# egorchistov/color-transfer

Measured on AMD Instinct MI355X. Metric: stereopairs/s at 1920×1080 (linear + dcmcs3di fwd), 1/2/4/8 GPU, higher is better.
Workload: dtype f32 (float32 I/O; float32 difference forms in both sweeps, float64 only in the per-frame statistics records); 1 GPU; configs[1]: methods.linear.color_transfer_between_images (Reinhard) on 1920x1080 synthetic float32 RGB pairs, HBM-resident; float32 arithmetic in both sweeps (difference forms, Lab within 5e-5 of the float64 reference; gate 1e-4); + per-frame psnr against resident ground truth; io_dtype=float32, height=1080, width=1920, lab_arithmetic=table

## Files before the change

color-transfer_amd/csrc/attention16.hip:

```cpp
#include <hip/hip_runtime.h>
#include <cstdint>
#include <cmath>
#include "ct_attention16.h"
#include "ct_env.h"
#include "ct_split16.h"

namespace ct {

static constexpr float kLog2eH = 1.4426950408889634f, kLn2H = 0.6931471805599453f;

constexpr int kSsRowH(int C) { return 2 * C + 16; }

__device__ __forceinline__ void xcd_order(int &bx, int &by) {
    bx = blockIdx.x; by = blockIdx.y;
    if (gridDim.z != 1) return;
    const unsigned int gx = gridDim.x, total = gx * gridDim.y, lin = by * gx + bx, full = total & ~7u;
    if (lin >= full) return;
    const unsigned int vid = (lin & 7u) * (full >> 3) + (lin >> 3);
    bx = (int)(vid % gx); by = (int)(vid / gx);
}

template <int C, int CV, bool MAP, bool IDX = false>
__global__ __launch_bounds__(256, 2) void attention16_tokens_kernel(const float *__restrict__ q, const float *__restrict__ k,
                                                                    const float *__restrict__ v, const int *__restrict__ region,
                                                                    const int *__restrict__ rowmap, float *__restrict__ out,
                                                                    float *__restrict__ stats, int L, float scale,
                                                                    float *__restrict__ part, long long kv_shift, long long kv_total,
                                                                    float *__restrict__ disp) {
    static_assert(!IDX || !MAP, "the expected index is built for the unmapped rows");
    constexpr bool PVS = CV >= 32;
    constexpr int NVT = PVS ? CV / 32 : 1;
    constexpr int KV4 = (32 * C / 4) / 256;
    constexpr int VV4 = PVS ? (32 * CV / 4) / 256 : 1;
    constexpr int SROW = kSsRowH(C);
    constexpr int VROWB = (CV * 2) % 256 == 0 ? CV * 2 + 64 : CV * 2;
// ... 158 lines not shown
    fetch_rows(jb);
    fetch(jb);
    fetch_rows(jb + 32);
    note_max();
    __syncthreads();
    stage();
    e_cur = e_stage;
    __syncthreads();
    for (int j0 = jb; j0 < je; j0 += 32) {
        const bool more = j0 + 32 < je;
        if (more) {
            fetch(j0 + 32);
            fetch_rows(j0 + 64);
        }
        f32x16 s;
#pragma unroll
        for (int r = 0; r < 16; ++r) s[r] = 0.f;
        {
            const unsigned char *kp = Ks + nl * SROW + 16 * hl;
            uint4 ac[2], an[2];
#pragma unroll
            for (int p = 0; p < 2; ++p) ac[p] = *reinterpret_cast<const uint4 *>(kp + p * 32 * SROW);
#pragma unroll
            for (int st = 0; st < C / 16; ++st) {
                if (st + 1 < C / 16) {
#pragma unroll
                    for (int p = 0; p < 2; ++p) an[p] = *reinterpret_cast<const uint4 *>(kp + p * 32 * SROW + 32 * (st + 1));
                }
                sp16_mfma3(s, ac, qf[st]);
#pragma unroll
                for (int p = 0; p < 2; ++p) ac[p] = an[p];
            }
        }
        const float f = Gs[0] * gq;
        if (region) {
            const float maskv = fmaxf((-100.0f * kLog2eH) * (Gs[1] * sq), -3.0e38f);
            int rk[16];
#pragma unroll
            for (int r = 0; r < 16; ++r) rk[r] = Rs[(r & 3) + 8 * (r >> 2) + 4 * hl];
#pragma unroll
            for (int r = 0; r < 16; ++r) s[r] += (rk[r] != qreg) ? maskv : 0.0f;
        }
        if (j0 + 32 > L) {
#pragma unroll
            for (int r = 0; r < 16; ++r) s[r] = (j0 + (r & 3) + 8 * (r >> 2) + 4 * hl < L) ? s[r] : -INFINITY;
        }
        float mx = s[0];
#pragma unroll
        for (int r = 1; r < 16; ++r) mx = fmaxf(mx, s[r]);
        mx = fmaxf(mx, __shfl_xor(mx, 32, 64));
        const float m_new = fmaxf(m_run, mx * f);
        const float corr = __builtin_amdgcn_exp2f(m_run - m_new);
        const float off = POFF - m_new;
        float psum = 0.f;
#pragma unroll
        for (int r = 0; r < 16; ++r) {
            const float p = __builtin_amdgcn_exp2f(fmaf(s[r], f, off));
            s[r] = p;
            psum += p;
        }
        psum += __shfl_xor(psum, 32, 64);
        l_run = l_run * corr + psum;
        m_run = m_new;
        if constexpr (IDX) {
            const float d0 = (float)(j0 + 4 * hl - qi);
            float asum = 0.f;
#pragma unroll
            for (int r = 0; r < 16; ++r) asum = fmaf(s[r], d0 + (float)((r & 3) + 8 * (r >> 2)), asum);
            asum += __shfl_xor(asum, 32, 64);
            a_run = a_run * corr + asum;
        }
        if constexpr (PVS) {
            const float ce = __builtin_amdgcn_ldexpf(corr, e_stage - e_cur);
            e_cur = e_stage;
#pragma unroll
            for (int j = 0; j < NVT; ++j)
#pragma unroll
                for (int r = 0; r < 16; ++r) o[j][r] *= ce;
            typedef short s16x4h __attribute__((ext_vector_type(4)));
            typedef __attribute__((address_space(3))) s16x4h *lds_s16x4;
            const unsigned char *vb = Vs + (4 * hl + ((lane & 15) >> 2)) * VROWB + (16 * ((lane >> 4) & 1) + 4 * (lane & 3)) * 2;
#pragma unroll
            for (int t = 0; t < 2; ++t) {
                const float x[8] = {s[8 * t], s[8 * t + 1], s[8 * t + 2], s[8 * t + 3], s[8 * t + 4], s[8 * t + 5], s[8 * t + 6], s[8 * t + 7]};
                uint4 pf[2];
                sp16_split2x8(x, pf[0], pf[1]);
#pragma unroll
                for (int j = 0; j < NVT; ++j) {
                    uint4 vf[2];
#pragma unroll
                    for (int p = 0; p < 2; ++p) {
                        const unsigned char *a = vb + (p * 32 + 16 * t) * VROWB + 64 * j;
                        const s16x4h lo = __builtin_amdgcn_ds_read_tr16_b64_v4i16((lds_s16x4)(a));
                        const s16x4h hi = __builtin_amdgcn_ds_read_tr16_b64_v4i16((lds_s16x4)(a + 8 * VROWB));
                        const uint2 l2 = __builtin_bit_cast(uint2, lo), h2 = __builtin_bit_cast(uint2, hi);
                        vf[p] = make_uint4(l2.x, l2.y, h2.x, h2.y);
                    }
                    sp16_mfma3(o[j], vf, pf);
                }
            }
        } else if constexpr (CV == 2) {
            const float *vs2 = reinterpret_cast<const float *>(Vs);
            float ax = 0.f, ay = 0.f;
#pragma unroll
            for (int r = 0; r < 16; ++r) {
                const float2 vv = *reinterpret_cast<const float2 *>(vs2 + ((r & 3) + 8 * (r >> 2) + 4 * hl) * 2);
                ax += s[r] * vv.x;
                ay += s[r] * vv.y;
            }
            ax += __shfl_xor(ax, 32, 64);
            ay += __shfl_xor(ay, 32, 64);
            o2x = o2x * corr + ax;
            o2y = o2y * corr + ay;
        }
        if (more) note_max();
        __syncthreads();
        if (more) {
            stage();
            __syncthreads();
        }
    }
    if (nsplit > 1) {
        float *pp = part + (((size_t)split * gridDim.y + b) * L + qclamp) * (CV + 2);
        if (qlive) {
            if constexpr (PVS) {
#pragma unroll
                for (int j = 0; j < NVT; ++j)
#pragma unroll
                    for (int r = 0; r < 16; ++r) pp[j * 32 + (r & 3) + 8 * (r >> 2) + 4 * hl] = __builtin_amdgcn_ldexpf(o[j][r], -e_cur - (int)POFF);
// ... 14 lines not shown
    }
    if constexpr (PVS) {
        if (qlive) {
            const float ie = __builtin_amdgcn_ldexpf(inv, -e_cur);
            float *op = out + row(qi) * CV;
#pragma unroll
            for (int j = 0; j < NVT; ++j)
#pragma unroll
                for (int r = 0; r < 16; r += 4)
                    *reinterpret_cast<float4 *>(op + j * 32 + 8 * (r >> 2) + 4 * hl) =
                        make_float4(o[j][r] * ie, o[j][r + 1] * ie, o[j][r + 2] * ie, o[j][r + 3] * ie);
        }
    } else if constexpr (CV == 2) {
        if (qlive && hl == 0) *reinterpret_cast<float2 *>(out + row(qi) * 2) = make_float2(o2x * inv, o2y * inv);
    }
}

template <int C>
__global__ __launch_bounds__(256, 2) void attention16_colsum_kernel(const float *__restrict__ q, const float *__restrict__ k,
                                                                    const float *__restrict__ stats, float *__restrict__ colsum, int L,
                                                                    float scale) {
    constexpr int QV4 = (32 * C / 4) / 256;
    constexpr int SROW = kSsRowH(C);
    __shared__ __attribute__((aligned(16))) unsigned char Qs[2 * 32 * SROW];
    __shared__ float2 Ms[32];
    __shared__ __attribute__((aligned(16))) float Mx[4];
    __shared__ float Gs[1];
    const int tid = threadIdx.x, lane = tid & 63, wave = tid >> 6, nl = lane & 31, hl = lane >> 5;
    int bxo, b;
    xcd_order(bxo, b);
// ... 60 lines not shown
            unsigned char *qd = Qs + qq * SROW + 8 * c4;
            *reinterpret_cast<uint2 *>(qd) = make_uint2(h0, h1);
            *reinterpret_cast<uint2 *>(qd + 32 * SROW) = make_uint2(l0, l1);
        }
        if (tid < 32) Ms[tid] = make_float2(mpre.x * kLog2eH, 1.0f / mpre.y);
    };
    float acc = 0.f;
    fetch(0);
    note_max();
    __syncthreads();
    stage();
    __syncthreads();
    for (int i0 = 0; i0 < L; i0 += 32) {
        const bool more = i0 + 32 < L;
        if (more) fetch(i0 + 32);
        f32x16 s;
#pragma unroll
        for (int r = 0; r < 16; ++r) s[r] = 0.f;
        const unsigned char *qp = Qs + nl * SROW + 16 * hl;
        uint4 ac[2], an[2];
#pragma unroll
        for (int p = 0; p < 2; ++p) ac[p] = *reinterpret_cast<const uint4 *>(qp + p * 32 * SROW);
#pragma unroll
        for (int st = 0; st < C / 16; ++st) {
            if (st + 1 < C / 16) {
#pragma unroll
                for (int p = 0; p < 2; ++p) an[p] = *reinterpret_cast<const uint4 *>(qp + p * 32 * SROW + 32 * (st + 1));
            }
            sp16_mfma3(s, ac, kf[st]);
#pragma unroll
            for (int p = 0; p < 2; ++p) ac[p] = an[p];
        }
        const float f = Gs[0] * gk;
        float2 ml[16];
#pragma unroll
        for (int r = 0; r < 16; ++r) ml[r] = Ms[(r & 3) + 8 * (r >> 2) + 4 * hl];
#pragma unroll
        for (int r = 0; r < 16; ++r) acc = fmaf(__builtin_amdgcn_exp2f(fmaf(s[r], f, -ml[r].x)), ml[r].y, acc);
        if (more) note_max();
        __syncthreads();
        if (more) {
            stage();
            __syncthreads();
        }
    }
    acc += __shfl_xor(acc, 32, 64);
    if (hl == 0 && kj < L) colsum[tb + kj] = acc;
}

bool attention16_enabled() {
    static const int on = env_int("CT_HIP_ATT16", 1);
    return on != 0;
}

void attention16_tokens128(const float *q, const float *k, const float *v, const int *region, const int *rowmap, float *out, int batch,
                           int len, int cv, float scale, int nsplit, float *ws, long long kv_shift, long long kv_total, hipStream_t s) {
    dim3 grid((len + 127) / 128, batch, nsplit);
    float *nostats = nullptr;
#define CT_ATT16(CVV, MAPPED) hipLaunchKernelGGL((attention16_tokens_kernel<128, CVV, MAPPED>), grid, dim3(256), 0, s, q, k, v, region, rowmap, out, nostats, len, scale, ws, kv_shift, kv_total, (float *)nullptr)
    if (cv == 128) { if (rowmap) CT_ATT16(128, true); else CT_ATT16(128, false); }
    else { if (rowmap) CT_ATT16(2, true); else CT_ATT16(2, false); }
#undef CT_ATT16
}

void attention16_rows64(const float *q, const float *k, const float *v, float *out, float *stats, int batch, int len, float scale,
                        hipStream_t s) {
    dim3 grid((len + 127) / 128, batch);
    const int *noreg = nullptr;
    if (v) hipLaunchKernelGGL((attention16_tokens_kernel<64, 96, false>), grid, dim3(256), 0, s, q, k, v, noreg, noreg, out, stats, len, scale, (float *)nullptr, 0LL, 0LL, (float *)nullptr);
    else hipLaunchKernelGGL((attention16_tokens_kernel<64, 0, false>), grid, dim3(256), 0, s, q, k, v, noreg, noreg, out, stats, len, scale, (float *)nullptr, 0LL, 0LL, (float *)nullptr);
}

void attention16_rows64_disp(const float *q, const float *k, const float *v, float *out, float *disp, int batch, int len, float scale,
                             hipStream_t s) {
    dim3 grid((len + 127) / 128, batch);
    const int *noreg = nullptr;
    float *nostats = nullptr;
    if (v) hipLaunchKernelGGL((attention16_tokens_kernel<64, 96, false, true>), grid, dim3(256), 0, s, q, k, v, noreg, noreg, out, nostats, len, scale, (float *)nullptr, 0LL, 0LL, disp);
    else hipLaunchKernelGGL((attention16_tokens_kernel<64, 0, false, true>), grid, dim3(256), 0, s, q, k, v, noreg, noreg, out, nostats, len, scale, (float *)nullptr, 0LL, 0LL, disp);
}

void attention16_colsum64(const float *q, const float *k, const float *stats, float *colsum, int batch, int len, float scale, hipStream_t s) {
    dim3 grid((len + 127) / 128, batch);
    hipLaunchKernelGGL((attention16_colsum_kernel<64>), grid, dim3(256), 0, s, q, k, stats, colsum, len, scale);
}

}
```

color-transfer_amd/csrc/attention_tokens.hip:

```cpp
#include "ct_common.h"
#include "ct_split.h"
#include "ct_attention16.h"

namespace ct {

template <bool TO_ROWS>
__global__ __launch_bounds__(256) void rows_transpose_kernel(const float *__restrict__ src, float *__restrict__ dst, int C, int H,
                                                             int W, long long nchw_bstride, int row_channels, int c0) {
    __shared__ float t[32][65];
    const int tid = threadIdx.x;
    const int x0 = blockIdx.x * 64;
    const int by = blockIdx.y, b = by / H, y = by - b * H;
    const size_t plane = (size_t)H * W;
    const float *nsrc = src;
    float *ndst = dst;
    const bool vec = (x0 + 64 <= W) && ((W & 3) == 0) && ((row_channels & 3) == 0) && ((c0 & 3) == 0) && ((nchw_bstride & 3) == 0) &&
                     (((reinterpret_cast<uintptr_t>(src) | reinterpret_cast<uintptr_t>(dst)) & 15) == 0);
    for (int cb = 0; cb < C; cb += 32) {
        const bool full = vec && (cb + 32 <= C);
        if (TO_ROWS) {
            const int c = tid >> 3, xs = (tid & 7) * 8;
            const float *p = nsrc + (size_t)b * nchw_bstride + (size_t)(cb + c) * plane + (size_t)y * W + x0 + xs;
            if (full) {
                const float4 a = reinterpret_cast<const float4 *>(p)[0], bb = reinterpret_cast<const float4 *>(p)[1];
// ... 561 lines not shown
    return CT_OK;
}

int ct_attention_colsum64_f32(const float *q, const float *k, const float *stats, float *colsum, int batch, int len, float scale,
                              void *stream) {
    if (!q || !k || !stats || !colsum || batch < 0 || len < 1) return CT_E_BADARG;
    if ((reinterpret_cast<uintptr_t>(q) | reinterpret_cast<uintptr_t>(k)) & 15) return CT_E_ALIGN;
    if (batch == 0) return CT_OK;
    dim3 grid((len + 127) / 128, batch);
    if (ct::attention16_enabled()) ct::attention16_colsum64(q, k, stats, colsum, batch, len, scale, (hipStream_t)stream);
    else hipLaunchKernelGGL((ct::attention_colsum_kernel<64>), grid, dim3(256), 0, (hipStream_t)stream, q, k, stats, colsum, len, scale);
    CT_CHECK_LAUNCH();
    return CT_OK;
}

}
```

color-transfer_amd/csrc/ct_attention16.h:

```cpp
#pragma once
#include <hip/hip_runtime.h>

namespace ct {

bool attention16_enabled();
void attention16_tokens128(const float *q, const float *k, const float *v, const int *region, const int *rowmap, float *out, int batch,
                           int len, int cv, float scale, int nsplit, float *ws, long long kv_shift, long long kv_total, hipStream_t s);
void attention16_rows64(const float *q, const float *k, const float *v, float *out, float *stats, int batch, int len, float scale,
                        hipStream_t s);
void attention16_rows64_disp(const float *q, const float *k, const float *v, float *out, float *disp, int batch, int len, float scale,
                             hipStream_t s);
void attention16_colsum64(const float *q, const float *k, const float *stats, float *colsum, int batch, int len, float scale, hipStream_t s);

}
```

color-transfer_amd/ct_hip/__init__.py:

```python
from ._core import (ACT_GELU, ACT_LEAKY, ACT_NONE, ACT_RELU, ACT_SIGMOID, ACT_SWISH, ACT_TANH, CT_ABI_VERSION,
                    CT_LAB_STATS_STRIDE, CT_RGB_STATS_STRIDE, CT_WS_IDT, CT_WS_LAB_STATS, CT_WS_REINHARD, CT_WS_REINHARD_PERSIST,
                    CT_WS_REINHARD_PSNR, CT_WS_RGB_MEANCOV, CtHipError, LIB_PATH, SIGNATURES, check, device_status, lib,
                    workspace, _stream)
from .linear import (CT_LAB_EXACT, CT_LAB_TABLE, affine3x3, lab_mode, lab_stats, mk, mk_coef, profile_events, reinhard,
                     reinhard_apply, reinhard_persist, reinhard_persist_supported, reinhard_psnr, reinhard_takes_persist,
                     rgb_meancov, set_lab_mode)
from .metrics import (CT_WS_FSIM, DISTORTIONS, distort_u8, fft2d_, frame_fsim, frame_icid, frame_psnr, frame_ssim, regrain,
                      _fsim_tables)
from .idt import IdtDebug, idt
from .resize_pack import CT_PACK_CHW, CT_PACK_HWC, PACK_LAYOUTS, bicubic_resize, bilinear_resize, pack_u8, resize_geometry
from .packing import (ConvSource, SplitOperands, pack_conv_weight, pack_conv_weight_split, pack_conv_weight_split16,
                      pack_conv_weight_wino16, pack_gconv_weight, pack_linear_weight_split, pack_linear_weight_ws16)
from .gmflow import (convex_upsample, eltwise, fb_check, flow_warp, instance_norm, local_attn_prop, local_corr_flow,
                     local_corr_softmax)
from .conv import (conv2d, conv2d_rows, conv_mode, conv_scratch_prepare, conv_stream_k_state, conv_wino, conv_ws16, gconv2d,
                   s2d_ok, set_conv_mode, set_conv_stream_k, set_conv_wino, set_conv_wino_form, set_conv_ws16, space_to_depth2,
                   _conv_scratch, _conv_split, _sk_cache)
from .linears import layernorm128, linear_layernorm128, linear_tokens, linear_tokens_multi, set_linear_ws16
from .attention import (attention_tokens, nchw_to_rows, nchw_to_tokens, pam_attend, pam_streaming, pam_streaming_rows, pam_valid,
                        pam_valid_rows, tokens_to_nchw)
from .unet import dwconv, gconv2d_pad, scale_planes_, se_gate, upsample2_concat
from .disparity import attention_rows64_index, pam_disp_fill, regress_disp
from .views import (CT_VIEW_ABMSE, CT_VIEW_GRAY, CT_VIEW_LABMSE, CT_VIEW_RGBMSE, abmse_view, chess_mix, flow_to_image, gray_view, labmse_view,
                    rgbmse_view, rgbssim_view)
from .png import INFLATE_STATUS, PNG_MAX_WIDTH, PNG_ROWS_PER_CHUNK, inflate, png_decode, png_deflate, png_geometry
from .augment import AUGMENT_KINDS, AUGMENT_MAX_OPS, AUGMENT_SAMPLE, augment_table, augment_u8, frame_losses
from .pam_losses import PAM_SWEEP_MAX_W, masked_l1_sums, pam_cycle_l1, pam_map_sweep
from . import _core


def __getattr__(name):
    if name == "_lib":
        return _core._lib
    raise AttributeError("module %r has no attribute %r" % (__name__, name))
```

color-transfer_amd/ct_hip/_core.py:

```python
import ctypes
import os
import threading
from typing import NamedTuple

import numpy as np
import torch

_HERE = os.path.dirname(os.path.abspath(__file__))
LIB_PATH = os.environ.get("CT_HIP_LIB") or os.path.join(_HERE, "libct_hip.so")

CT_ABI_VERSION = 9
CT_LAB_STATS_STRIDE = 8
CT_RGB_STATS_STRIDE = 16
CT_WS_LAB_STATS, CT_WS_RGB_MEANCOV, CT_WS_REINHARD, CT_WS_IDT, CT_WS_REINHARD_PSNR, CT_WS_REINHARD_PERSIST = 0, 1, 2, 3, 4, 5

_c_i64 = ctypes.c_int64
_c_int = ctypes.c_int
_c_p = ctypes.c_void_p
_c_sz = ctypes.c_size_t
_c_ll = ctypes.c_longlong
_c_f = ctypes.c_float

ACT_NONE, ACT_LEAKY, ACT_RELU, ACT_SIGMOID, ACT_TANH, ACT_SWISH, ACT_GELU = 0, 1, 2, 3, 4, 5, 6

# ... 18 lines not shown
        with _lock:
            if _lib is None:
                if not os.path.exists(LIB_PATH):
                    raise CtHipError(
                        "HIP library %s not found: build it with `python -c 'import __graft_entry__ as g; g.build()'` "
                        "or `make -C color-transfer_amd/csrc`; this package has no CPU fallback" % LIB_PATH)
                handle = ctypes.CDLL(LIB_PATH)
                for name, (res, args) in SIGNATURES.items():
                    fn = getattr(handle, name)
                    fn.restype = res
                    fn.argtypes = args
                got = handle.ct_abi_version()
                if got != CT_ABI_VERSION:
                    raise CtHipError("%s reports ABI version %d, this binding needs %d: rebuild with `make -C color-transfer_amd/csrc`"
                                     % (LIB_PATH, got, CT_ABI_VERSION))
                _lib = handle
    return _lib


def check(rc):
    if rc != 0:
        raise CtHipError("libct_hip: %s (code %d)" % (lib().ct_error_string(rc).decode(), rc))


def _stream():
    return ctypes.c_void_p(torch.cuda.current_stream().cuda_stream)


def _check_device(t):
    if t.device.index is not None and t.device.index != torch.cuda.current_device():
# ... 117 lines not shown
```

color-transfer_amd/ct_hip/attention.py:

```python
import ctypes

import torch

from ._core import (CtHipError, SIGNATURES, _c_f, _c_int, _c_ll, _c_p, _c_sz, _check_device, _f32c, _nchw_bstride, _opt, _ptr, _stream,
                    check, lib, workspace)

SIGNATURES.update({
    "ct_pam_workspace_bytes": (_c_sz, [_c_int, _c_int, _c_int]),
    "ct_pam_attend_f32": (_c_int, [_c_p, _c_p, _c_p, _c_p, _c_p, _c_p, _c_p, _c_int, _c_int, _c_int, _c_int, _c_int, _c_p]),
    "ct_pam_valid_f32": (_c_int, [_c_p, _c_p, _c_p, _c_p, _c_p, _c_int, _c_int, _c_int, _c_int, _c_p, _c_sz, _c_p]),
    "ct_attention_workspace_bytes": (ctypes.c_size_t, [_c_int, _c_int, _c_int, _c_int]),
    "ct_attention_tokens_f32": (_c_int, [_c_p, _c_p, _c_p, _c_p, _c_p, _c_p, _c_int, _c_int, _c_int, _c_f, _c_int, _c_p,
                                         ctypes.c_size_t, ctypes.c_longlong, _c_p]),
    "ct_nchw_to_rows_f32": (_c_int, [_c_p, _c_p, _c_int, _c_int, _c_int, _c_int, _c_ll, _c_int, _c_int, _c_p]),
    "ct_rows_to_nchw_f32": (_c_int, [_c_p, _c_p, _c_int, _c_int, _c_int, _c_int, _c_ll, _c_int, _c_int, _c_p]),
    "ct_attention_rows64_f32": (_c_int, [_c_p, _c_p, _c_p, _c_p, _c_p, _c_int, _c_int, _c_f, _c_p]),
    "ct_attention_colsum64_f32": (_c_int, [_c_p, _c_p, _c_p, _c_p, _c_int, _c_int, _c_f, _c_p]),
})


def pam_attend(q, k, v, rgb, want_att=False):
    for t in (q, k, v, rgb):
        if t.is_cuda:
            _check_device(t)
        if not t.is_cuda or t.dtype != torch.float32 or not t.is_contiguous():
            raise CtHipError("pam_attend needs contiguous float32 CUDA tensors")
    n, c, h, w = q.shape
    cv = v.shape[1]
    out_v = torch.empty_like(v)
    out_rgb = torch.empty_like(rgb)
    att = torch.empty((n, h, w, w), dtype=torch.float32, device=q.device) if want_att else None
    check(lib().ct_pam_attend_f32(_ptr(q), _ptr(k), _ptr(v), _ptr(rgb), _ptr(out_v), _ptr(out_rgb),
                                  _ptr(att) if att is not None else _c_p(0), n, c, cv, h, w, _stream()))
# ... 125 lines not shown
```

include/ct_hip.h:

```cpp
#ifndef CT_HIP_H
#define CT_HIP_H

#include <stddef.h>
#include <stdint.h>

#ifdef __cplusplus
extern "C" {
#endif

#define CT_OK 0
#define CT_E_BADARG (-1)
#define CT_E_WORKSPACE (-2)
#define CT_E_ALIGN (-3)

#define CT_ABI_VERSION 9

#define CT_LAB_STATS_STRIDE 8
#define CT_RGB_STATS_STRIDE 16

enum ct_workspace_kind {
    CT_WS_LAB_STATS = 0,
    CT_WS_RGB_MEANCOV = 1,
    CT_WS_REINHARD = 2,
    CT_WS_IDT = 3,
// ... 118 lines not shown
int ct_conv2d_split_rows_f32(const float *in, const void *wp_split, const float *bias, float *out_rows, int n, int cin, int cout,
                             int h, int w, int kh, int kw, long long in_bstride, int rows_channels, int rows_c0, int act,
                             int f16, int w_exp, void *stream);

int ct_conv1x1_rows_f32(const float *in, const float *weight, const float *bias, float *out_rows, int n, int cin, int cout, int h, int w,
                        long long in_bstride, int rows_channels, int rows_c0, int act, void *stream);

int ct_conv3x3_ws16_f32(const float *in, const void *wp16, int w_exp, const float *bias, const float *residual, float *out, int n,
                        int cin, int cout, int h, int w, long long in_bstride, long long out_bstride, long long res_bstride, int act,
                        int clamp, void *stream);

int ct_conv3x3_wino16_f32(const float *in, const void *wq16, int w_exp, const float *bias, const float *residual, float *out, int n,
                          int cin, int cout, int h, int w, long long in_bstride, long long out_bstride, long long res_bstride, int act,
                          int clamp, void *stream);
int ct_set_conv_wino_form(int form);

int ct_pam_attend_f32(const float *q, const float *k, const float *v, const float *rgb,
                      float *out_v, float *out_rgb, float *att, int n, int c, int cv, int h, int w,
                      void *stream);
size_t ct_pam_workspace_bytes(int n, int h, int w);
int ct_pam_valid_f32(const float *q, const float *k, float *valid, float *colsum, float *att,
                     int n, int c, int h, int w, void *ws, size_t ws_bytes, void *stream);

int ct_gconv2d_f32(const float *in, const float *wp, const float *bias, float *out, int n, int cin,
                   int cout, int h, int w, int kh, int kw, int stride, int pad_h, int pad_w,
                   long long in_bstride, long long out_bstride, int act, void *stream);
size_t ct_instance_norm_workspace_bytes(int planes);
int ct_instance_norm_f32(const float *x, const float *skip, float *y, int planes, int plane, float eps,
                         int mode, void *ws, size_t ws_bytes, void *stream);
int ct_space_to_depth2_f32(const float *in, float *out, int n, int c, int h, int w, long long in_bstride, void *stream);
// ... 132 lines not shown
```

Measured before the change: 42890 stereopairs/s.

## Add 8-wave rows64 attention and colsum kernels sharing K/V tiles

Adds 512-thread workgroup variants of the rows64 attention (plain and disparity-index) and colsum kernels. Each block holds 256 query rows across 8 waves and stages 64-key K/V tiles as two 32-key sub-tiles with per-sub-tile scaling exponents, which halves the K/V staging traffic and barrier count per query row. The variant is the default and can be switched back through an env var or setter. It also skips the output rescale when no lane's correction factor differs from one. In exchange it uses one block per CU with more LDS, which risks lower occupancy and longer barrier stalls.

```diff
diff --git a/color-transfer_amd/csrc/attention16.hip b/color-transfer_amd/csrc/attention16.hip
--- a/color-transfer_amd/csrc/attention16.hip
+++ b/color-transfer_amd/csrc/attention16.hip
@@ -1,4 +1,5 @@
 #include <hip/hip_runtime.h>
+#include <atomic>
 #include <cstdint>
 #include <cmath>
 #include "ct_attention16.h"
@@ -19,6 +20,115 @@
     const unsigned int vid = (lin & 7u) * (full >> 3) + (lin >> 3);
     bx = (int)(vid % gx); by = (int)(vid / gx);
 }
+
+constexpr int att16_nvt(int CV) { return CV >= 32 ? CV / 32 : 1; }
+
+template <int C>
+__device__ __forceinline__ void att16_scores(f32x16 &s, const unsigned char *Kt, const uint4 (&qf)[C / 16][2], int nl, int hl) {
+    constexpr int SROW = kSsRowH(C);
+#pragma unroll
+    for (int r = 0; r < 16; ++r) s[r] = 0.f;
+    const unsigned char *kp = Kt + nl * SROW + 16 * hl;
+    uint4 ac[2], an[2];
+#pragma unroll
+    for (int p = 0; p < 2; ++p) ac[p] = *reinterpret_cast<const uint4 *>(kp + p * 32 * SROW);
+#pragma unroll
+    for (int st = 0; st < C / 16; ++st) {
+        if (st + 1 < C / 16) {
+#pragma unroll
+            for (int p = 0; p < 2; ++p) an[p] = *reinterpret_cast<const uint4 *>(kp + p * 32 * SROW + 32 * (st + 1));
+        }
+        sp16_mfma3(s, ac, qf[st]);
+#pragma unroll
+        for (int p = 0; p < 2; ++p) ac[p] = an[p];
+    }
+}
+
+template <int CV, bool IDX, bool LAZY>
+__device__ __forceinline__ void att16_softmax_pv(f32x16 &s, float f, int j0, int L, int qi, int lane, const unsigned char *Vt, int e_stage,
+                                                 int &e_cur, float &m_run, float &l_run, float &a_run, f32x16 (&o)[att16_nvt(CV)],
+                                                 float &o2x, float &o2y) {
+    constexpr bool PVS = CV >= 32;
+    constexpr int NVT = att16_nvt(CV);
+    constexpr int VROWB = (CV * 2) % 256 == 0 ? CV * 2 + 64 : CV * 2;
+    constexpr float POFF = PVS ? 15.0f : 0.0f;
+    const int hl = lane >> 5;
+    if (j0 + 32 > L) {
+#pragma unroll
+        for (int r = 0; r < 16; ++r) s[r] = (j0 + (r & 3) + 8 * (r >> 2) + 4 * hl < L) ? s[r] : -INFINITY;
+    }
+    float mx = s[0];
+#pragma unroll
+    for (int r = 1; r < 16; ++r) mx = fmaxf(mx, s[r]);
+    mx = fmaxf(mx, __shfl_xor(mx, 32, 64));
+    const float m_new = fmaxf(m_run, mx * f);
+    const float corr = __builtin_amdgcn_exp2f(m_run - m_new);
+    const float off = POFF - m_new;
+    float psum = 0.f;
+#pragma unroll
+    for (int r = 0; r < 16; ++r) {
+        const float p = __builtin_amdgcn_exp2f(fmaf(s[r], f, off));
+        s[r] = p;
+        psum += p;
+    }
+    psum += __shfl_xor(psum, 32, 64);
+    l_run = l_run * corr + psum;
+    m_run = m_new;
+    if constexpr (IDX) {
+        const float d0 = (float)(j0 + 4 * hl - qi);
+        float asum = 0.f;
+#pragma unroll
+        for (int r = 0; r < 16; ++r) asum = fmaf(s[r], d0 + (float)((r & 3) + 8 * (r >> 2)), asum);
+        asum += __shfl_xor(asum, 32, 64);
+        a_run = a_run * corr + asum;
+    }
+    if constexpr (PVS) {
+        const float ce = __builtin_amdgcn_ldexpf(corr, e_stage - e_cur);
+        e_cur = e_stage;
+        if (!LAZY || __builtin_amdgcn_ballot_w64(ce != 1.0f) != 0) {
+#pragma unroll
+            for (int j = 0; j < NVT; ++j)
+#pragma unroll
+                for (int r = 0; r < 16; ++r) o[j][r] *= ce;
+        }
+        typedef short s16x4h __attribute__((ext_vector_type(4)));
+        typedef __attribute__((address_space(3))) s16x4h *lds_s16x4;
+        const unsigned char *vb = Vt + (4 * hl + ((lane & 15) >> 2)) * VROWB + (16 * ((lane >> 4) & 1) + 4 * (lane & 3)) * 2;
+#pragma unroll
+        for (int t = 0; t < 2; ++t) {
+            const float x[8] = {s[8 * t], s[8 * t + 1], s[8 * t + 2], s[8 * t + 3], s[8 * t + 4], s[8 * t + 5], s[8 * t + 6], s[8 * t + 7]};
+            uint4 pf[2];
+            sp16_split2x8(x, pf[0], pf[1]);
+#pragma unroll
+            for (int j = 0; j < NVT; ++j) {
+                uint4 vf[2];
+#pragma unroll
+                for (int p = 0; p < 2; ++p) {
+                    const unsigned char *a = vb + (p * 32 + 16 * t) * VROWB + 64 * j;
+                    const s16x4h lo = __builtin_amdgcn_ds_read_tr16_b64_v4i16((lds_s16x4)(a));
+                    const s16x4h hi = __builtin_amdgcn_ds_read_tr16_b64_v4i16((lds_s16x4)(a + 8 * VROWB));
+                    const uint2 l2 = __builtin_bit_cast(uint2, lo), h2 = __builtin_bit_cast(uint2, hi);
+                    vf[p] = make_uint4(l2.x, l2.y, h2.x, h2.y);
+                }
+                sp16_mfma3(o[j], vf, pf);
+            }
+        }
+    } else if constexpr (CV == 2) {
+        const float *vs2 = reinterpret_cast<const float *>(Vt);
+        float ax = 0.f, ay = 0.f;
+#pragma unroll
+        for (int r = 0; r < 16; ++r) {
+            const float2 vv = *reinterpret_cast<const float2 *>(vs2 + ((r & 3) + 8 * (r >> 2) + 4 * hl) * 2);
+            ax += s[r] * vv.x;
+            ay += s[r] * vv.y;
+        }
+        ax += __shfl_xor(ax, 32, 64);
+        ay += __shfl_xor(ay, 32, 64);
+        o2x = o2x * corr + ax;
+        o2y = o2y * corr + ay;
+    }
+}
+
 
 template <int C, int CV, bool MAP, bool IDX = false>
 __global__ __launch_bounds__(256, 2) void attention16_tokens_kernel(const float *__restrict__ q, const float *__restrict__ k,
@@ -207,24 +317,7 @@
             fetch_rows(j0 + 64);
         }
         f32x16 s;
-#pragma unroll
-        for (int r = 0; r < 16; ++r) s[r] = 0.f;
-        {
-            const unsigned char *kp = Ks + nl * SROW + 16 * hl;
-            uint4 ac[2], an[2];
-#pragma unroll
-            for (int p = 0; p < 2; ++p) ac[p] = *reinterpret_cast<const uint4 *>(kp + p * 32 * SROW);
-#pragma unroll
-            for (int st = 0; st < C / 16; ++st) {
-                if (st + 1 < C / 16) {
-#pragma unroll
-                    for (int p = 0; p < 2; ++p) an[p] = *reinterpret_cast<const uint4 *>(kp + p * 32 * SROW + 32 * (st + 1));
-                }
-                sp16_mfma3(s, ac, qf[st]);
-#pragma unroll
-                for (int p = 0; p < 2; ++p) ac[p] = an[p];
-            }
-        }
+        att16_scores<C>(s, Ks, qf, nl, hl);
         const float f = Gs[0] * gq;
         if (region) {
             const float maskv = fmaxf((-100.0f * kLog2eH) * (Gs[1] * sq), -3.0e38f);
@@ -234,78 +327,7 @@
 #pragma unroll
             for (int r = 0; r < 16; ++r) s[r] += (rk[r] != qreg) ? maskv : 0.0f;
         }
-        if (j0 + 32 > L) {
-#pragma unroll
-            for (int r = 0; r < 16; ++r) s[r] = (j0 + (r & 3) + 8 * (r >> 2) + 4 * hl < L) ? s[r] : -INFINITY;
-        }
-        float mx = s[0];
-#pragma unroll
-        for (int r = 1; r < 16; ++r) mx = fmaxf(mx, s[r]);
-        mx = fmaxf(mx, __shfl_xor(mx, 32, 64));
-        const float m_new = fmaxf(m_run, mx * f);
-        const float corr = __builtin_amdgcn_exp2f(m_run - m_new);
-        const float off = POFF - m_new;
-        float psum = 0.f;
-#pragma unroll
-        for (int r = 0; r < 16; ++r) {
-            const float p = __builtin_amdgcn_exp2f(fmaf(s[r], f, off));
-            s[r] = p;
-            psum += p;
-        }
-        psum += __shfl_xor(psum, 32, 64);
-        l_run = l_run * corr + psum;
-        m_run = m_new;
-        if constexpr (IDX) {
-            const float d0 = (float)(j0 + 4 * hl - qi);
-            float asum = 0.f;
-#pragma unroll
-            for (int r = 0; r < 16; ++r) asum = fmaf(s[r], d0 + (float)((r & 3) + 8 * (r >> 2)), asum);
-            asum += __shfl_xor(asum, 32, 64);
-            a_run = a_run * corr + asum;
-        }
-        if constexpr (PVS) {
-            const float ce = __builtin_amdgcn_ldexpf(corr, e_stage - e_cur);
-            e_cur = e_stage;
-#pragma unroll
-            for (int j = 0; j < NVT; ++j)
-#pragma unroll
-                for (int r = 0; r < 16; ++r) o[j][r] *= ce;
-            typedef short s16x4h __attribute__((ext_vector_type(4)));
-            typedef __attribute__((address_space(3))) s16x4h *lds_s16x4;
-            const unsigned char *vb = Vs + (4 * hl + ((lane & 15) >> 2)) * VROWB + (16 * ((lane >> 4) & 1) + 4 * (lane & 3)) * 2;
-#pragma unroll
-            for (int t = 0; t < 2; ++t) {
-                const float x[8] = {s[8 * t], s[8 * t + 1], s[8 * t + 2], s[8 * t + 3], s[8 * t + 4], s[8 * t + 5], s[8 * t + 6], s[8 * t + 7]};
-                uint4 pf[2];
-                sp16_split2x8(x, pf[0], pf[1]);
-#pragma unroll
-                for (int j = 0; j < NVT; ++j) {
-                    uint4 vf[2];
-#pragma unroll
-                    for (int p = 0; p < 2; ++p) {
-                        const unsigned char *a = vb + (p * 32 + 16 * t) * VROWB + 64 * j;
-                        const s16x4h lo = __builtin_amdgcn_ds_read_tr16_b64_v4i16((lds_s16x4)(a));
-                        const s16x4h hi = __builtin_amdgcn_ds_read_tr16_b64_v4i16((lds_s16x4)(a + 8 * VROWB));
-                        const uint2 l2 = __builtin_bit_cast(uint2, lo), h2 = __builtin_bit_cast(uint2, hi);
-                        vf[p] = make_uint4(l2.x, l2.y, h2.x, h2.y);
-                    }
-                    sp16_mfma3(o[j], vf, pf);
-                }
-            }
-        } else if constexpr (CV == 2) {
-            const float *vs2 = reinterpret_cast<const float *>(Vs);
-            float ax = 0.f, ay = 0.f;
-#pragma unroll
-            for (int r = 0; r < 16; ++r) {
-                const float2 vv = *reinterpret_cast<const float2 *>(vs2 + ((r & 3) + 8 * (r >> 2) + 4 * hl) * 2);
-                ax += s[r] * vv.x;
-                ay += s[r] * vv.y;
-            }
-            ax += __shfl_xor(ax, 32, 64);
-            ay += __shfl_xor(ay, 32, 64);
-            o2x = o2x * corr + ax;
-            o2y = o2y * corr + ay;
-        }
+        att16_softmax_pv<CV, IDX, C == 64>(s, f, j0, L, qi, lane, Vs, e_stage, e_cur, m_run, l_run, a_run, o, o2x, o2y);
         if (more) note_max();
         __syncthreads();
         if (more) {
@@ -350,6 +372,18 @@
     } else if constexpr (CV == 2) {
         if (qlive && hl == 0) *reinterpret_cast<float2 *>(out + row(qi) * 2) = make_float2(o2x * inv, o2y * inv);
     }
+}
+
+template <int C>
+__device__ __forceinline__ void att16_colsum_tile(float &acc, const unsigned char *Qt, const float2 *Mt, float f, const uint4 (&kf)[C / 16][2],
+                                                  int nl, int hl) {
+    f32x16 s;
+    att16_scores<C>(s, Qt, kf, nl, hl);
+    float2 ml[16];
+#pragma unroll
+    for (int r = 0; r < 16; ++r) ml[r] = Mt[(r & 3) + 8 * (r >> 2) + 4 * hl];
+#pragma unroll
+    for (int r = 0; r < 16; ++r) acc = fmaf(__builtin_amdgcn_exp2f(fmaf(s[r], f, -ml[r].x)), ml[r].y, acc);
 }
 
 template <int C>
@@ -440,33 +474,320 @@
     for (int i0 = 0; i0 < L; i0 += 32) {
         const bool more = i0 + 32 < L;
         if (more) fetch(i0 + 32);
-        f32x16 s;
-#pragma unroll
-        for (int r = 0; r < 16; ++r) s[r] = 0.f;
-        const unsigned char *qp = Qs + nl * SROW + 16 * hl;
-        uint4 ac[2], an[2];
-#pragma unroll
-        for (int p = 0; p < 2; ++p) ac[p] = *reinterpret_cast<const uint4 *>(qp + p * 32 * SROW);
-#pragma unroll
-        for (int st = 0; st < C / 16; ++st) {
-            if (st + 1 < C / 16) {
-#pragma unroll
-                for (int p = 0; p < 2; ++p) an[p] = *reinterpret_cast<const uint4 *>(qp + p * 32 * SROW + 32 * (st + 1));
-            }
-            sp16_mfma3(s, ac, kf[st]);
-#pragma unroll
-            for (int p = 0; p < 2; ++p) ac[p] = an[p];
-        }
-        const float f = Gs[0] * gk;
-        float2 ml[16];
-#pragma unroll
-        for (int r = 0; r < 16; ++r) ml[r] = Ms[(r & 3) + 8 * (r >> 2) + 4 * hl];
-#pragma unroll
-        for (int r = 0; r < 16; ++r) acc = fmaf(__builtin_amdgcn_exp2f(fmaf(s[r], f, -ml[r].x)), ml[r].y, acc);
+        att16_colsum_tile<C>(acc, Qs, Ms, Gs[0] * gk, kf, nl, hl);
         if (more) note_max();
         __syncthreads();
         if (more) {
             stage();
+            __syncthreads();
+        }
+    }
+    acc += __shfl_xor(acc, 32, 64);
+    if (hl == 0 && kj < L) colsum[tb + kj] = acc;
+}
+
+constexpr int kWg8Threads = 512, kWg8Rows = 256;
+constexpr int kAtt16DefaultWaves = 8;
+
+__device__ __forceinline__ float att16_amax4(const float4 &t) { return fmaxf(fmaxf(fabsf(t.x), fabsf(t.y)), fmaxf(fabsf(t.z), fabsf(t.w))); }
+
+template <int CV, bool IDX>
+__global__ __launch_bounds__(kWg8Threads, 1) void attention16_rows64_wg8_kernel(const float *__restrict__ q, const float *__restrict__ k,
+                                                                                const float *__restrict__ v, float *__restrict__ out,
+                                                                                float *__restrict__ stats, int L, float scale,
+                                                                                float *__restrict__ disp) {
+    constexpr int C = 64;
+    constexpr bool PVS = CV >= 32;
+    constexpr int NVT = att16_nvt(CV);
+    constexpr int KV4 = (64 * C / 4) / kWg8Threads;
+    constexpr int VV4 = PVS ? (64 * CV / 4) / kWg8Threads : 1;
+    constexpr int VSPLIT = 32 * CV / 4;
+    static_assert(KV4 == 2, "sub-tile i of K is float4 i of a thread");
+    static_assert(!PVS || ((64 * CV / 4) % kWg8Threads == 0 && VSPLIT % 64 == 0), "a wave's float4 of V lie in one sub-tile");
+    constexpr int SROW = kSsRowH(C);
+    constexpr int VROWB = (CV * 2) % 256 == 0 ? CV * 2 + 64 : CV * 2;
+    static_assert(!PVS || ((VROWB / 4) % 64 == 16 || (VROWB / 4) % 64 == 48), "V image rows must not share banks");
+    constexpr int KSUB = 2 * 32 * SROW, VSUB = 2 * 32 * VROWB;
+    constexpr float POFF = PVS ? 15.0f : 0.0f;
+    __shared__ __attribute__((aligned(16))) unsigned char Ks[2 * KSUB];
+    __shared__ __attribute__((aligned(16))) unsigned char Vs[PVS ? 2 * VSUB : 256];
+    __shared__ __attribute__((aligned(16))) int Mx[2][4];
+    __shared__ float Gs[2];
+    const int tid = threadIdx.x, lane = tid & 63, wave = __builtin_amdgcn_readfirstlane(tid >> 6), nl = lane & 31, hl = lane >> 5;
+    int bxo, b;
+    xcd_order(bxo, b);
+    const int q0 = (bxo * 8 + wave) * 32;
+    const bool wlive = q0 < L;
+    const size_t tb = (size_t)b * L;
+    const int qi = q0 + nl;
+    const bool qlive = qi < L;
+    const int qclamp = qlive ? qi : L - 1;
+    if (tid < 8) (&Mx[0][0])[tid] = 0;
+    uint4 qf[C / 16][2];
+    float gq;
+    {
+        const float qs = scale * kLog2eH;
+        const float *qp = q + (tb + qclamp) * C + 8 * hl;
+        float x[C / 16][8];
+        float amax = 0.f;
+#pragma unroll
+        for (int st = 0; st < C / 16; ++st) {
+            const float4 t0 = *reinterpret_cast<const float4 *>(qp + 16 * st), t1 = *reinterpret_cast<const float4 *>(qp + 16 * st + 4);
+            x[st][0] = t0.x * qs; x[st][1] = t0.y * qs; x[st][2] = t0.z * qs; x[st][3] = t0.w * qs;
+            x[st][4] = t1.x * qs; x[st][5] = t1.y * qs; x[st][6] = t1.z * qs; x[st][7] = t1.w * qs;
+#pragma unroll
+            for (int j = 0; j < 8; ++j) amax = fmaxf(amax, fabsf(x[st][j]));
+        }
+        amax = fmaxf(amax, __shfl_xor(amax, 32, 64));
+        const int eq = sp16_scale_exp(amax, 0);
+        const float sq = sp16_pow2i(eq);
+        gq = sp16_pow2i(-eq);
+#pragma unroll
+        for (int st = 0; st < C / 16; ++st) {
+#pragma unroll
+            for (int j = 0; j < 8; ++j) x[st][j] *= sq;
+            sp16_split2x8(x[st], qf[st][0], qf[st][1]);
+        }
+    }
+
+    float4 kpre[KV4], vpre[VV4];
+    auto fetch = [&](int j0) {
+#pragma unroll
+        for (int i = 0; i < KV4; ++i) {
+            const int f = tid + i * kWg8Threads, key = f / (C / 4), c4 = f - key * (C / 4);
+            kpre[i] = (j0 + key < L) ? *reinterpret_cast<const float4 *>(k + (tb + j0 + key) * C + 4 * c4) : make_float4(0.f, 0.f, 0.f, 0.f);
+        }
+        if constexpr (PVS) {
+#pragma unroll
+            for (int i = 0; i < VV4; ++i) {
+                const int f = tid + i * kWg8Threads, key = f / (CV / 4), c4 = f - key * (CV / 4);
+                vpre[i] = (j0 + key < L) ? *reinterpret_cast<const float4 *>(v + (tb + j0 + key) * CV + 4 * c4) : make_float4(0.f, 0.f, 0.f, 0.f);
+            }
+        }
+    };
+    auto note_max = [&](int par) {
+        float mk0 = att16_amax4(kpre[0]), mk1 = att16_amax4(kpre[1]), mv0 = 0.f, mv1 = 0.f;
+        if constexpr (PVS) {
+#pragma unroll
+            for (int i = 0; i < VV4; ++i) {
+                const bool sub1 = wave * 64 + i * kWg8Threads >= VSPLIT;
+                const float a = att16_amax4(vpre[i]);
+                mv0 = sub1 ? mv0 : fmaxf(mv0, a);
+                mv1 = sub1 ? fmaxf(mv1, a) : mv1;
+            }
+        }
+        mk0 = wave_max_nonneg_lane63(mk0);
+        mk1 = wave_max_nonneg_lane63(mk1);
+        if constexpr (PVS) { mv0 = wave_max_nonneg_lane63(mv0); mv1 = wave_max_nonneg_lane63(mv1); }
+        if (lane == 63) {
+            atomicMax(&Mx[par][0], __float_as_int(mk0));
+            atomicMax(&Mx[par][2], __float_as_int(mk1));
+            if constexpr (PVS) { atomicMax(&Mx[par][1], __float_as_int(mv0)); atomicMax(&Mx[par][3], __float_as_int(mv1)); }
+        }
+    };
+    int e_sub[2] = {100, 100}, e_cur = 100;
+    auto stage = [&](int par) {
+        const int4 mm = *reinterpret_cast<const int4 *>(Mx[par]);
+        const int ek[2] = {__builtin_amdgcn_readfirstlane(sp16_scale_exp(__int_as_float(mm.x), 0)),
+                           __builtin_amdgcn_readfirstlane(sp16_scale_exp(__int_as_float(mm.z), 0))};
+        if (tid == 0) {
+            Gs[0] = sp16_pow2i(-ek[0]); Gs[1] = sp16_pow2i(-ek[1]);
+            *reinterpret_cast<int4 *>(Mx[par ^ 1]) = make_int4(0, 0, 0, 0);
+        }
+#pragma unroll
+        for (int i = 0; i < KV4; ++i) {
+            const int f = tid + i * kWg8Threads, key = f / (C / 4) - 32 * i, c4 = f & (C / 4 - 1);
+            const float sk = sp16_pow2i(ek[i]);
+            unsigned int h0, l0, h1, l1;
+            sp16_split2x2(kpre[i].x * sk, kpre[i].y * sk, h0, l0);
+            sp16_split2x2(kpre[i].z * sk, kpre[i].w * sk, h1, l1);
+            unsigned char *kd = Ks + i * KSUB + key * SROW + 8 * c4;
+            *reinterpret_cast<uint2 *>(kd) = make_uint2(h0, h1);
+            *reinterpret_cast<uint2 *>(kd + 32 * SROW) = make_uint2(l0, l1);
+        }
+        if constexpr (PVS) {
+            e_sub[0] = __builtin_amdgcn_readfirstlane(min(e_sub[1], sp16_scale_exp(__int_as_float(mm.y), 100)));
+            e_sub[1] = __builtin_amdgcn_readfirstlane(min(e_sub[0], sp16_scale_exp(__int_as_float(mm.w), 100)));
+#pragma unroll
+            for (int i = 0; i < VV4; ++i) {
+                const int f = tid + i * kWg8Threads, key = f / (CV / 4), c4 = f - key * (CV / 4);
+                const bool sub1 = wave * 64 + i * kWg8Threads >= VSPLIT;
+                const float sv = sp16_pow2i(sub1 ? e_sub[1] : e_sub[0]);
+                unsigned int h0, l0, h1, l1;
+                sp16_split2x2(vpre[i].x * sv, vpre[i].y * sv, h0, l0);
+                sp16_split2x2(vpre[i].z * sv, vpre[i].w * sv, h1, l1);
+                unsigned char *vd = Vs + (sub1 ? VSUB - 32 * VROWB : 0) + key * VROWB + 8 * c4;
+                *reinterpret_cast<uint2 *>(vd) = make_uint2(h0, h1);
+                *reinterpret_cast<uint2 *>(vd + 32 * VROWB) = make_uint2(l0, l1);
+            }
+        }
+    };
+
+    float m_run = -INFINITY, l_run = 0.f, a_run = 0.f;
+    f32x16 o[NVT];
+    float o2x = 0.f, o2y = 0.f;
+    if constexpr (PVS) {
+#pragma unroll
+        for (int j = 0; j < NVT; ++j)
+#pragma unroll
+            for (int r = 0; r < 16; ++r) o[j][r] = 0.f;
+    }
+    fetch(0);
+    __syncthreads();
+    note_max(0);
+    __syncthreads();
+    stage(0);
+    e_cur = e_sub[0];
+    __syncthreads();
+    int par = 0;
+    for (int j0 = 0; j0 < L; j0 += 64) {
+        const bool more = j0 + 64 < L;
+        if (more) fetch(j0 + 64);
+        if (wlive) {
+#pragma unroll
+            for (int sub = 0; sub < 2; ++sub) {
+                if (sub == 0 || j0 + 32 < L) {
+                    f32x16 s;
+                    att16_scores<C>(s, Ks + sub * KSUB, qf, nl, hl);
+                    const float f = Gs[sub] * gq;
+                    att16_softmax_pv<CV, IDX, true>(s, f, j0 + 32 * sub, L, qi, lane, Vs + (PVS ? sub * VSUB : 0), e_sub[sub], e_cur, m_run, l_run, a_run, o,
+                                                    o2x, o2y);
+                }
+            }
+        }
+        par ^= 1;
+        if (more) note_max(par);
+        __syncthreads();
+        if (more) {
+            stage(par);
+            __syncthreads();
+        }
+    }
+    if (!qlive) return;
+    const float inv = 1.0f / l_run;
+    if constexpr (IDX) {
+        if (hl == 0) disp[tb + qi] = -a_run / l_run;
+    }
+    if (stats && hl == 0) {
+        stats[(tb + qi) * 2] = m_run * kLn2H;
+        stats[(tb + qi) * 2 + 1] = __builtin_amdgcn_ldexpf(l_run, -(int)POFF);
+    }
+    if constexpr (PVS) {
+        const float ie = __builtin_amdgcn_ldexpf(inv, -e_cur);
+        float *op = out + (tb + qi) * CV;
+#pragma unroll
+        for (int j = 0; j < NVT; ++j)
+#pragma unroll
+            for (int r = 0; r < 16; r += 4)
+                *reinterpret_cast<float4 *>(op + j * 32 + 8 * (r >> 2) + 4 * hl) =
+                    make_float4(o[j][r] * ie, o[j][r + 1] * ie, o[j][r + 2] * ie, o[j][r + 3] * ie);
+    }
+}
+
+__global__ __launch_bounds__(kWg8Threads, 1) void attention16_colsum64_wg8_kernel(const float *__restrict__ q, const float *__restrict__ k,
+                                                                                  const float *__restrict__ stats, float *__restrict__ colsum,
+                                                                                  int L, float scale) {
+    constexpr int C = 64;
+    constexpr int QV4 = (64 * C / 4) / kWg8Threads;
+    static_assert(QV4 == 2, "sub-tile i of Q is float4 i of a thread");
+    constexpr int SROW = kSsRowH(C);
+    constexpr int QSUB = 2 * 32 * SROW;
+    __shared__ __attribute__((aligned(16))) unsigned char Qs[2 * QSUB];
+    __shared__ float2 Ms[64];
+    __shared__ __attribute__((aligned(8))) int Mx[2][2];
+    __shared__ float Gs[2];
+    const int tid = threadIdx.x, lane = tid & 63, wave = __builtin_amdgcn_readfirstlane(tid >> 6), nl = lane & 31, hl = lane >> 5;
+    int bxo, b;
+    xcd_order(bxo, b);
+    const int j0 = (bxo * 8 + wave) * 32;
+    const bool wlive = j0 < L;
+    const size_t tb = (size_t)b * L;
+    const int kj = j0 + nl;
+    if (tid < 4) (&Mx[0][0])[tid] = 0;
+    uint4 kf[C / 16][2];
+    float gk;
+    {
+        const float qs = scale * kLog2eH;
+        const float *kp = k + (tb + (kj < L ? kj : L - 1)) * C + 8 * hl;
+        float x[C / 16][8];
+        float amax = 0.f;
+#pragma unroll
+        for (int st = 0; st < C / 16; ++st) {
+            const float4 t0 = *reinterpret_cast<const float4 *>(kp + 16 * st), t1 = *reinterpret_cast<const float4 *>(kp + 16 * st + 4);
+            x[st][0] = t0.x * qs; x[st][1] = t0.y * qs; x[st][2] = t0.z * qs; x[st][3] = t0.w * qs;
+            x[st][4] = t1.x * qs; x[st][5] = t1.y * qs; x[st][6] = t1.z * qs; x[st][7] = t1.w * qs;
+#pragma unroll
+            for (int j = 0; j < 8; ++j) amax = fmaxf(amax, fabsf(x[st][j]));
+        }
+        amax = fmaxf(amax, __shfl_xor(amax, 32, 64));
+        const int ek = sp16_scale_exp(amax, 0);
+        const float sk = sp16_pow2i(ek);
+        gk = sp16_pow2i(-ek);
+#pragma unroll
+        for (int st = 0; st < C / 16; ++st) {
+#pragma unroll
+            for (int j = 0; j < 8; ++j) x[st][j] *= sk;
+            sp16_split2x8(x[st], kf[st][0], kf[st][1]);
+        }
+    }
+    float4 qpre[QV4];
+    float2 mpre = make_float2(0.f, 0.f);
+    auto fetch = [&](int i0) {
+#pragma unroll
+        for (int i = 0; i < QV4; ++i) {
+            const int f = tid + i * kWg8Threads, qq = f / (C / 4), c4 = f - qq * (C / 4);
+            qpre[i] = (i0 + qq < L) ? *reinterpret_cast<const float4 *>(q + (tb + i0 + qq) * C + 4 * c4) : make_float4(0.f, 0.f, 0.f, 0.f);
+        }
+        if (tid < 64) {
+            mpre = (i0 + tid < L) ? *reinterpret_cast<const float2 *>(stats + (tb + i0 + tid) * 2) : make_float2(INFINITY, INFINITY);
+        }
+    };
+    auto note_max = [&](int par) {
+        const float m0 = wave_max_nonneg_lane63(att16_amax4(qpre[0])), m1 = wave_max_nonneg_lane63(att16_amax4(qpre[1]));
+        if (lane == 63) { atomicMax(&Mx[par][0], __float_as_int(m0)); atomicMax(&Mx[par][1], __float_as_int(m1)); }
+    };
+    auto stage = [&](int par) {
+        const int2 mm = *reinterpret_cast<const int2 *>(Mx[par]);
+        const int eq[2] = {__builtin_amdgcn_readfirstlane(sp16_scale_exp(__int_as_float(mm.x), 0)),
+                           __builtin_amdgcn_readfirstlane(sp16_scale_exp(__int_as_float(mm.y), 0))};
+        if (tid == 0) {
+            Gs[0] = sp16_pow2i(-eq[0]); Gs[1] = sp16_pow2i(-eq[1]);
+            *reinterpret_cast<int2 *>(Mx[par ^ 1]) = make_int2(0, 0);
+        }
+#pragma unroll
+        for (int i = 0; i < QV4; ++i) {
+            const int f = tid + i * kWg8Threads, qq = f / (C / 4) - 32 * i, c4 = f & (C / 4 - 1);
+            const float sqv = sp16_pow2i(eq[i]);
+            unsigned int h0, l0, h1, l1;
+            sp16_split2x2(qpre[i].x * sqv, qpre[i].y * sqv, h0, l0);
+            sp16_split2x2(qpre[i].z * sqv, qpre[i].w * sqv, h1, l1);
+            unsigned char *qd = Qs + i * QSUB + qq * SROW + 8 * c4;
+            *reinterpret_cast<uint2 *>(qd) = make_uint2(h0, h1);
+            *reinterpret_cast<uint2 *>(qd + 32 * SROW) = make_uint2(l0, l1);
+        }
+        if (tid < 64) Ms[tid] = make_float2(mpre.x * kLog2eH, 1.0f / mpre.y);
+    };
+    float acc = 0.f;
+    fetch(0);
+    __syncthreads();
+    note_max(0);
+    __syncthreads();
+    stage(0);
+    __syncthreads();
+    int par = 0;
+    for (int i0 = 0; i0 < L; i0 += 64) {
+        const bool more = i0 + 64 < L;
+        if (more) fetch(i0 + 64);
+        if (wlive) {
+#pragma unroll
+            for (int sub = 0; sub < 2; ++sub)
+                if (sub == 0 || i0 + 32 < L) att16_colsum_tile<C>(acc, Qs + sub * QSUB, Ms + 32 * sub, Gs[sub] * gk, kf, nl, hl);
+        }
+        par ^= 1;
+        if (more) note_max(par);
+        __syncthreads();
+        if (more) {
+            stage(par);
             __syncthreads();
         }
     }
@@ -489,8 +810,22 @@
 #undef CT_ATT16
 }
 
+static std::atomic<int> g_att16_waves{kAtt16DefaultWaves};
+int attention16_waves() { return g_att16_waves.load(std::memory_order_relaxed); }
+bool attention16_set_waves(int waves) {
+    if (waves != 4 && waves != 8) return false;
+    g_att16_waves.store(waves, std::memory_order_relaxed);
+    return true;
+}
+
 void attention16_rows64(const float *q, const float *k, const float *v, float *out, float *stats, int batch, int len, float scale,
                         hipStream_t s) {
+    if (attention16_waves() == 8) {
+        dim3 grid((len + kWg8Rows - 1) / kWg8Rows, batch);
+        if (v) hipLaunchKernelGGL((attention16_rows64_wg8_kernel<96, false>), grid, dim3(kWg8Threads), 0, s, q, k, v, out, stats, len, scale, (float *)nullptr);
+        else hipLaunchKernelGGL((attention16_rows64_wg8_kernel<0, false>), grid, dim3(kWg8Threads), 0, s, q, k, v, out, stats, len, scale, (float *)nullptr);
+        return;
+    }
     dim3 grid((len + 127) / 128, batch);
     const int *noreg = nullptr;
     if (v) hipLaunchKernelGGL((attention16_tokens_kernel<64, 96, false>), grid, dim3(256), 0, s, q, k, v, noreg, noreg, out, stats, len, scale, (float *)nullptr, 0LL, 0LL, (float *)nullptr);
@@ -499,14 +834,25 @@
 
 void attention16_rows64_disp(const float *q, const float *k, const float *v, float *out, float *disp, int batch, int len, float scale,
                              hipStream_t s) {
+    float *nostats = nullptr;
+    if (attention16_waves() == 8) {
+        dim3 grid((len + kWg8Rows - 1) / kWg8Rows, batch);
+        if (v) hipLaunchKernelGGL((attention16_rows64_wg8_kernel<96, true>), grid, dim3(kWg8Threads), 0, s, q, k, v, out, nostats, len, scale, disp);
+        else hipLaunchKernelGGL((attention16_rows64_wg8_kernel<0, true>), grid, dim3(kWg8Threads), 0, s, q, k, v, out, nostats, len, scale, disp);
+        return;
+    }
     dim3 grid((len + 127) / 128, batch);
     const int *noreg = nullptr;
-    float *nostats = nullptr;
     if (v) hipLaunchKernelGGL((attention16_tokens_kernel<64, 96, false, true>), grid, dim3(256), 0, s, q, k, v, noreg, noreg, out, nostats, len, scale, (float *)nullptr, 0LL, 0LL, disp);
     else hipLaunchKernelGGL((attention16_tokens_kernel<64, 0, false, true>), grid, dim3(256), 0, s, q, k, v, noreg, noreg, out, nostats, len, scale, (float *)nullptr, 0LL, 0LL, disp);
 }
 
 void attention16_colsum64(const float *q, const float *k, const float *stats, float *colsum, int batch, int len, float scale, hipStream_t s) {
+    if (attention16_waves() == 8) {
+        dim3 grid((len + kWg8Rows - 1) / kWg8Rows, batch);
+        hipLaunchKernelGGL(attention16_colsum64_wg8_kernel, grid, dim3(kWg8Threads), 0, s, q, k, stats, colsum, len, scale);
+        return;
+    }
     dim3 grid((len + 127) / 128, batch);
     hipLaunchKernelGGL((attention16_colsum_kernel<64>), grid, dim3(256), 0, s, q, k, stats, colsum, len, scale);
 }
diff --git a/color-transfer_amd/csrc/attention_tokens.hip b/color-transfer_amd/csrc/attention_tokens.hip
--- a/color-transfer_amd/csrc/attention_tokens.hip
+++ b/color-transfer_amd/csrc/attention_tokens.hip
@@ -599,4 +599,8 @@
     return CT_OK;
 }
 
-}
+int ct_set_attention16_waves(int waves) { return ct::attention16_set_waves(waves) ? CT_OK : CT_E_BADARG; }
+
+int ct_get_attention16_waves(void) { return ct::attention16_waves(); }
+
+}
diff --git a/color-transfer_amd/csrc/ct_attention16.h b/color-transfer_amd/csrc/ct_attention16.h
--- a/color-transfer_amd/csrc/ct_attention16.h
+++ b/color-transfer_amd/csrc/ct_attention16.h
@@ -4,6 +4,8 @@
 namespace ct {
 
 bool attention16_enabled();
+int attention16_waves();
+bool attention16_set_waves(int waves);
 void attention16_tokens128(const float *q, const float *k, const float *v, const int *region, const int *rowmap, float *out, int batch,
                            int len, int cv, float scale, int nsplit, float *ws, long long kv_shift, long long kv_total, hipStream_t s);
 void attention16_rows64(const float *q, const float *k, const float *v, float *out, float *stats, int batch, int len, float scale,
diff --git a/color-transfer_amd/ct_hip/__init__.py b/color-transfer_amd/ct_hip/__init__.py
--- a/color-transfer_amd/ct_hip/__init__.py
+++ b/color-transfer_amd/ct_hip/__init__.py
@@ -17,8 +17,8 @@
                    s2d_ok, set_conv_mode, set_conv_stream_k, set_conv_wino, set_conv_wino_form, set_conv_ws16, space_to_depth2,
                    _conv_scratch, _conv_split, _sk_cache)
 from .linears import layernorm128, linear_layernorm128, linear_tokens, linear_tokens_multi, set_linear_ws16
-from .attention import (attention_tokens, nchw_to_rows, nchw_to_tokens, pam_attend, pam_streaming, pam_streaming_rows, pam_valid,
-                        pam_valid_rows, tokens_to_nchw)
+from .attention import (attention_tokens, get_attention16_waves, nchw_to_rows, nchw_to_tokens, pam_attend, pam_streaming,
+                        pam_streaming_rows, pam_valid, pam_valid_rows, set_attention16_waves, tokens_to_nchw)
 from .unet import dwconv, gconv2d_pad, scale_planes_, se_gate, upsample2_concat
 from .disparity import attention_rows64_index, pam_disp_fill, regress_disp
 from .views import (CT_VIEW_ABMSE, CT_VIEW_GRAY, CT_VIEW_LABMSE, CT_VIEW_RGBMSE, abmse_view, chess_mix, flow_to_image, gray_view, labmse_view,
diff --git a/color-transfer_amd/ct_hip/_core.py b/color-transfer_amd/ct_hip/_core.py
--- a/color-transfer_amd/ct_hip/_core.py
+++ b/color-transfer_amd/ct_hip/_core.py
@@ -56,6 +56,11 @@
                 if got != CT_ABI_VERSION:
                     raise CtHipError("%s reports ABI version %d, this binding needs %d: rebuild with `make -C color-transfer_amd/csrc`"
                                      % (LIB_PATH, got, CT_ABI_VERSION))
+                waves = os.environ.get("CT_HIP_ATT16_WAVES")
+                if waves:
+                    rc = handle.ct_set_attention16_waves(int(waves))
+                    if rc != 0:
+                        raise CtHipError("CT_HIP_ATT16_WAVES=%s: the rows64 attention has a 4-wave and an 8-wave form" % waves)
                 _lib = handle
     return _lib
 
diff --git a/color-transfer_amd/ct_hip/attention.py b/color-transfer_amd/ct_hip/attention.py
--- a/color-transfer_amd/ct_hip/attention.py
+++ b/color-transfer_amd/ct_hip/attention.py
@@ -16,7 +16,17 @@
     "ct_rows_to_nchw_f32": (_c_int, [_c_p, _c_p, _c_int, _c_int, _c_int, _c_int, _c_ll, _c_int, _c_int, _c_p]),
     "ct_attention_rows64_f32": (_c_int, [_c_p, _c_p, _c_p, _c_p, _c_p, _c_int, _c_int, _c_f, _c_p]),
     "ct_attention_colsum64_f32": (_c_int, [_c_p, _c_p, _c_p, _c_p, _c_int, _c_int, _c_f, _c_p]),
+    "ct_set_attention16_waves": (_c_int, [_c_int]),
+    "ct_get_attention16_waves": (_c_int, []),
 })
+
+
+def set_attention16_waves(waves):
+    check(lib().ct_set_attention16_waves(int(waves)))
+
+
+def get_attention16_waves():
+    return int(lib().ct_get_attention16_waves())
 
 
 def pam_attend(q, k, v, rgb, want_att=False):
diff --git a/include/ct_hip.h b/include/ct_hip.h
--- a/include/ct_hip.h
+++ b/include/ct_hip.h
@@ -156,6 +156,9 @@
                           int cin, int cout, int h, int w, long long in_bstride, long long out_bstride, long long res_bstride, int act,
                           int clamp, void *stream);
 int ct_set_conv_wino_form(int form);
+
+int ct_set_attention16_waves(int waves);
+int ct_get_attention16_waves(void);
 
 int ct_pam_attend_f32(const float *q, const float *k, const float *v, const float *rgb,
                       float *out_v, float *out_rgb, float *att, int n, int c, int cv, int h, int w,
```

Result: no change. 42880 stereopairs/s, median of 2 (-0.0%).
